# inhavl-shlee/AFI-GAN

Hardware: AMD Instinct MI355X
Metric: stage1_G+D_step_images_per_s (higher is better)
Workload: dtype f32 via f16x3: two scaled fp16 pieces per operand, three f16 MFMAs per product, fp32 accumulate (tensors fp32)

## Files before the change

afigan_amd/csrc/afi_launch.h:

```cpp
#pragma once
#include "afi_common.h"

int afi_launch_pix_gemm(const AfiPixGemm& p, int b_rc, hipStream_t st);
int afi_launch_gemm_tn(const float* Q, const float* V, float* dU, int planes, long long rows_per_plane, int M, int N, hipStream_t st, bool deterministic = false);
int afi_launch_gemm_nt(const float* A, const float* B, float* C, int planes, long long rows_per_plane, int N, int K, hipStream_t st);
int afi_launch_split_bf16_tiles(const float* B, void* out, int planes, int N, int K, int split, hipStream_t st);
int afi_launch_gemm_nt_bf16_dma(const float* A, const void* Bsplit, float* C, int planes, long long rows_per_plane, int N, int K, int split, hipStream_t st);
int afi_launch_gemm_tn_bf16(const float* Q, const float* V, float* dU, int planes, long long rows_per_plane, int M, int N, int split, hipStream_t st, bool deterministic = false);
int afi_launch_split_f16_tiles(const float* B, void* out, int planes, int N, int K, hipStream_t st, int wkind = 0);
int afi_f16_image_begin(void* out, hipStream_t st);
float* afi_f16_image_wmax(void* out);
long long afi_f16_image_bytes(int planes, int N, int K);
int afi_launch_absmax_planes(const float* X, long long per_plane, int planes, float* out, hipStream_t st);
AfiF16Bound afi_f16_bound(const float* amax, int kind);
int afi_launch_gemm_nt_f16x3(const float* A, const void* Bimg, float* C, int planes, long long rows_per_plane, int N, int K, const AfiF16Bound& ab, hipStream_t st,
                             bool a_pre = false, long long nt256_min_tiles = 512, bool local_sums = false);
int afi_launch_gemm_tn_f16x3(const float* Q, const float* V, float* dU, int planes, long long rows_per_plane, int M, int N, const AfiF16Bound& qb, const AfiF16Bound& vb,
                             hipStream_t st, bool pre = false, bool deterministic = false);
int afi_launch_wgrad_gemm(const AfiWgradGemm& p, hipStream_t st);
int afi_launch_wgrad_gemm_group(const AfiWgradGemm* probs, int n, int wide, hipStream_t st);
int afi_launch_wgrad_gemm_group6(const AfiWgradGemm* probs, int n, hipStream_t st);
int afi_launch_pix_gemm_group(const AfiPixGemm* probs, int n, int b_rc, hipStream_t st);

long long afi_wk6_image_bytes(int Ncols, int Ck, int ntaps, int nKphase);
int afi_launch_wk6_images(const AfiWk6ImgJob* jobs, int n, hipStream_t st, const AfiWk6Side* side = nullptr, const AfiWk6ConvT* ct = nullptr);
int afi_launch_rdb_chain6(const AfiChain6& c, hipStream_t st);
int afi_launch_pix_gemm_sk(const AfiPixGemm& p, int b_rc, hipStream_t st);
int afi_launch_pix_gemm_wk_group(const AfiPixGemm* probs, int n, int b_rc, hipStream_t st);
int afi_launch_wgrad_group(const AfiWgradGemm* probs, int n, int wide, hipStream_t st);
int afi_launch_wgrad6_group(const AfiWgradGemm* probs, int n, hipStream_t st);

int afi_launch_nchw_to_nhwc(const float* in, float* out, int N, int C, int P, hipStream_t st);
int afi_launch_cast_to_f32_nhwc(const void* in, int dt, int N, int C, int H, int W, long long sN, long long sC, long long sH, long long sW, float* out,
                                hipStream_t st);
int afi_launch_cast_from_f32_nhwc(const AfiView& in, int N, int H, int W, int C, void* out, int dt, hipStream_t st);

int afi_launch_colsum_group(const AfiColsumProb* probs, int n, hipStream_t st);
int afi_launch_nhwc_to_nchw(const float* in, float* out, int N, int C, int P, hipStream_t st);
int afi_launch_convT_pack(const float* W, float* Wp, int Cin, int Cout, hipStream_t st);
int afi_launch_convT_unpack_grad(const float* dWp, float* dW, int Cin, int Cout, hipStream_t st);
int afi_launch_rdb_wgrad_unpack(const float* dWp, float* const dw[4], int C, int G, float alpha, hipStream_t st);
int afi_launch_rdb_wgrad_unpack_multi(const float* dWp, long long stride, float* const (*dw)[4], int nblocks, int C, int G, float alpha, hipStream_t st);
int afi_launch_g_bwd_tail(const AfiColsumProb* cs, int n_cs, const float* dWpT, float* dWT, int Cin, int Cout,
                          const float* dWp, long long stride, float* const (*dw)[4], int nblocks, int C, int G, float alpha, hipStream_t st);
int afi_launch_rdb_xpart_pack(const float* const w[4], float* out, int C, int G, hipStream_t st);
int afi_launch_lrelu_slice(AfiView v, int N, int H, int W, int nch, hipStream_t st);
int afi_launch_bn_stats(const float* x, long long P, int C, float* mean, float* invstd, float* var_out, float* running_mean,
                        float* running_var, float* scratch, hipStream_t st, long long* num_batches_tracked = nullptr, float eps = -1.f,
                        float momentum = -1.f, bool fp64 = true);
int afi_launch_bn_stats_from_partials(const double* partial, int rows, long long P, int C, float* mean, float* invstd, float* var_out, float* running_mean,
                                      float* running_var, hipStream_t st, long long* num_batches_tracked = nullptr, float eps = -1.f, float momentum = -1.f);
int afi_launch_view_absmax(AfiView x, int N, int H, int W, int C, float* amax, hipStream_t st);
int afi_launch_bn_act_amax(const float* mm, int rows, int C, const float* mean, const float* invstd, const float* gamma, const float* beta, float slope,
                           float* amax, hipStream_t st);
int afi_launch_bn_apply_lrelu(const float* x, float* y, const float* mean, const float* invstd, const float* gamma, const float* beta,
                              long long P, int C, hipStream_t st, float slope = AFI_LRELU_SLOPE, float* amax = nullptr);
int afi_launch_bn_bwd(const float* g, const float* x, float* dx, const float* mean, const float* invstd, const float* gamma, float* dgamma,
                      float* dbeta, float gscale, long long P, int C, float* scratch, hipStream_t st, const float* mask_beta = nullptr,
                      float slope = AFI_LRELU_SLOPE, float* amax = nullptr);
int afi_launch_colsum_accum(const float* g, long long P, int C, long long ld, float alpha, float* db, float* scratch, hipStream_t st);
int afi_launch_bn_bwd_sums(const float* g, const float* x, const float* mean, const float* invstd, float* dgamma, float* dbeta, float* sums2C, long long P, int C,
                           float* scratch, hipStream_t st);
int afi_launch_bn_bwd_apply(const float* g, const float* x, float* dx, const float* mean, const float* invstd, const float* gamma, const float* sums2C, long long P,
                            long long P_total, int C, hipStream_t st);
int afi_launch_stencil9_sum(const float* d9, int ld, const float* bias, float* out, int N, int H, int W, hipStream_t st);
int afi_launch_stencil9_scatter(const float* dlogit, float* dd9, int ld, int N, int H, int W, hipStream_t st);
int afi_launch_bn_bwd_from_partials(const double* partial, int rows, const float* g, const float* x, float* dx, const float* mean, const float* invstd,
                                    const float* gamma, float* dgamma, float* dbeta, float gscale, long long P, int C, float* scratch, hipStream_t st,
                                    const float* mask_beta, float slope, float* amax);
extern "C" long long afi_disc_tail_scratch_floats(int C);
int afi_launch_disc_tail_fwd(const float* x, const AfiBnLoad* bn, float slope, const float* w3, float* d9, long long P, int C, hipStream_t st);
int afi_launch_disc_tail_bwd(const float* x, const float* dd9, const AfiBnLoad bn, float slope, const float* w3, float* dx, float* dgamma, float* dbeta, float* dw3,
                             long long P, int C, float* scratch, float* amax, hipStream_t st);
int afi_launch_bce_logits(const float* z, long long n, float target, float lscale, float* loss, float gscale, float* dz, hipStream_t st);
int afi_launch_l1(AfiView a, AfiView b, int N, int h, int w, int C, int Ha, int Wa, float lscale, float* loss, float gscale, float* da,
// ... 32 lines not shown
```

afigan_amd/csrc/igemm.hip:

```cpp
#include "afi_common.h"
#include "afi_launch.h"

#define AFI_BK 32
#define AFI_LDK (AFI_BK + 4)


__device__ __attribute__((aligned(16))) float afi_zeros[4] = {0.f, 0.f, 0.f, 0.f};

#include "afi_epilogue.h"

template <bool POST>
__global__ __launch_bounds__(256) void afi_pix_splitk_epilogue_kernel(const AfiPixGemm p) {
    const int HW = p.H * p.W;
    const long long M = (long long)p.N * HW;
    const int ldp = (p.Ncols + 3) & ~3;
    const int C_F4 = ldp >> 2;
    const long long total = M * C_F4;
    for (long long it = (long long)blockIdx.x * 256 + threadIdx.x; it < total; it += (long long)gridDim.x * 256) {
        const long long m = it / C_F4;
        const int col = (int)(it - m * C_F4) * 4;
        f32x4 v = {0.f, 0.f, 0.f, 0.f};
        const float* src = p.partial + m * ldp + col;
        const long long slab = M * ldp;
        int ks = 0;
// ... 479 lines not shown
    const long long ldn = p.N;
    if (use_atomic) {
#pragma unroll
        for (int mi = 0; mi < MI; ++mi)
#pragma unroll
            for (int r = 0; r < 16; ++r) {
                const int row = m0 + MI * ((r & 3) + 8 * (r >> 2) + 4 * lh) + mi;
                atomicAdd(out + (long long)row * ldn + n0 + wn * 32 + lr, acc[mi][r]);
            }
    } else {
        float old[MI][16];
#pragma unroll
        for (int mi = 0; mi < MI; ++mi)
#pragma unroll
            for (int r = 0; r < 16; ++r) {
                const int row = m0 + MI * ((r & 3) + 8 * (r >> 2) + 4 * lh) + mi;
                old[mi][r] = out[(long long)row * ldn + n0 + wn * 32 + lr];
            }
#pragma unroll
        for (int mi = 0; mi < MI; ++mi)
#pragma unroll
            for (int r = 0; r < 16; ++r) {
                const int row = m0 + MI * ((r & 3) + 8 * (r >> 2) + 4 * lh) + mi;
                out[(long long)row * ldn + n0 + wn * 32 + lr] = old[mi][r] + acc[mi][r];
            }
    }
}

#include <vector>
#include <atomic>
#include <mutex>
namespace {
struct ProfRec { hipEvent_t a, b; int kind; double flops; long long m; int n, k, split, planes; };
struct ProfState {
    std::atomic<bool> on{false};
    std::mutex mu;
    std::vector<ProfRec> recs;
    std::vector<hipEvent_t> pool;
    size_t used = 0;
} g_prof;
const char* kKindNames[] = {
    "pix_gemm<128x128,KC,linear> (1x1 / ragged-map / non-aligned Winograd GEMMs)", "pix_gemm<128x64,KC>", "pix_gemm<128x32,KC>", "pix_gemm<64x64,KC>",
    "pix_gemm<128x128,RC,linear> (conv dgrad, mid-size / ragged maps)", "pix_gemm<128x64,RC>", "pix_gemm<128x32,RC>", "pix_gemm<64x64,RC>",
    "wgrad_gemm<128x128>", "wgrad_gemm<64x128>", "wgrad_gemm<32x128>",
    "pix_gemm<128x128,KC,halo> (conv fwd)", "pix_gemm<128x128,RC,halo> (conv dgrad)",
    "gemm_nt<128x128> (batched Winograd GEMM)", "gemm_tn<128x128> (Winograd weight-gradient GEMM)",
    "pix_gemm_wk (small-map pixel GEMM, K split inside the block; grouped launches included)",
    "wgrad_group (grouped weight gradients of a small-map backward pass)",
    "gemm_nt_bf16<128x128> (batched Winograd GEMM on the bf16 MFMA: bf16x6 / bf16x3 / bf16 operands, fp32 accumulate)",
    "gemm_tn_bf16<128x128> (Winograd weight-gradient GEMM on the bf16 MFMA: bf16x6 / bf16x3 / bf16 operands, fp32 accumulate)",
    "wgrad_group6 (grouped weight gradients of a small-map backward pass on the bf16 MFMA, bf16x6 operands, fp32 accumulate)",
    "pix_gemm_wk6 (small-map pixel GEMM on the bf16 MFMA, bf16x6 operands on pre-split weight images, fp32 accumulate; grouped launches included)",
    "gemm_nt_f16x3 (batched Winograd GEMM on the f16 MFMA, 256x256 tiles where the grid fills the chip and 128x128 below: two scaled fp16 pieces per operand, three products, fp32 accumulate)",
    "gemm_tn_f16x3<128x128> (Winograd weight-gradient GEMM on the f16 MFMA: two scaled fp16 pieces per operand, three products, fp32 accumulate)"};
constexpr int kNumKinds = 23;
hipEvent_t prof_event() {
    if (g_prof.used == g_prof.pool.size()) {
        hipEvent_t e;
        (void)hipEventCreate(&e);
        g_prof.pool.push_back(e);
    }
    return g_prof.pool[g_prof.used++];
}
struct ProfScope {
    hipStream_t st; int kind; double flops; hipEvent_t a{};
    long long m = 0; int n = 0, k = 0, split = 1, planes = 1;
    ProfScope(hipStream_t s, int kd, double f) : st(s), kind(kd), flops(f) {
        if (g_prof.on) { std::lock_guard<std::mutex> lk(g_prof.mu); a = prof_event(); (void)hipEventRecord(a, st); started = true; }
    }
    bool live = true, started = false;
    void cancel() { live = false; }
    ~ProfScope() {
        if (started && live) { std::lock_guard<std::mutex> lk(g_prof.mu); hipEvent_t b = prof_event(); (void)hipEventRecord(b, st); g_prof.recs.push_back({a, b, kind, flops, m, n, k, split, planes}); }
    }
};
}

extern "C" int afi_profile_enable(int on) {
    std::lock_guard<std::mutex> lk(g_prof.mu);
    if (on) { g_prof.recs.clear(); g_prof.used = 0; }
    g_prof.on = on != 0;
    return AFI_OK;
}
extern "C" int afi_profile_num_kinds(void) { return kNumKinds; }
extern "C" const char* afi_profile_kind_name(int kind) { return (kind >= 0 && kind < kNumKinds) ? kKindNames[kind] : ""; }
extern "C" int afi_profile_get(int kind, double* out) {
    out[0] = out[1] = out[2] = 0.0;
    for (const ProfRec& r : g_prof.recs) {
        if (r.kind != kind) continue;
        if (hipEventSynchronize(r.b) != hipSuccess) return AFI_ERR_LAUNCH;
        float ms = 0.f;
        if (hipEventElapsedTime(&ms, r.a, r.b) != hipSuccess) return AFI_ERR_LAUNCH;
        out[0] += 1.0; out[1] += ms; out[2] += r.flops;
    }
    return AFI_OK;
}

#include <stdio.h>
extern "C" int afi_profile_dump(const char* path) {
    FILE* f = fopen(path, "w");
    if (!f) return AFI_ERR_BAD_ARG;
    fprintf(f, "kind,rows,cols,k,split,planes,ms,tflops\n");
    for (const ProfRec& r : g_prof.recs) {
        float ms = 0.f;
        if (hipEventSynchronize(r.b) != hipSuccess || hipEventElapsedTime(&ms, r.a, r.b) != hipSuccess) { fclose(f); return AFI_ERR_LAUNCH; }
        fprintf(f, "\"%s\",%lld,%d,%d,%d,%d,%.4f,%.2f\n", kKindNames[r.kind], r.m, r.n, r.k, r.split, r.planes, ms, ms > 0.f ? r.flops / (ms * 1e-3) / 1e12 : 0.0);
    }
    fclose(f);
// ... 224 lines not shown
            const long long blocks = tiles * s2;
            if (blocks < 2 * slots && s2 < maxsplit) continue;
            if (blocks > AFI_TN_MAX_ROUNDS * slots && best >= 0.0) break;
            const long long rounds = (blocks + slots - 1) / slots;
            const double fill = (double)blocks / (double)(rounds * slots);
            if (fill > best + 1e-3) { best = fill; splitK = s2; }
        }
    }
    if (deterministic) splitK = 1;
    int kper = (int)((rows_per_plane + splitK - 1) / splitK);
    kper = ((kper + 31) / 32) * 32;
    splitK = (int)((rows_per_plane + kper - 1) / kper);
    AfiGemmTN g{Q, V, dU, rows_per_plane, planes, M, N};
    ProfScope prof(st, 22, 2.0 * (double)rows_per_plane * planes * M * N);
    prof.m = (long long)M * planes; prof.n = N; prof.k = (int)rows_per_plane; prof.split = splitK; prof.planes = planes;
    if (pre) hipLaunchKernelGGL(afi_gemm_tn_f16x3_pre_kernel, dim3((unsigned)tiles, splitK), dim3(64 * AFI_TN_WAVES), (unsigned)AFI_TN_RING * 4u * 4096u, st, g, qb, vb, ntm, ntn, kper);
    else hipLaunchKernelGGL(afi_gemm_tn_f16x3_kernel, dim3((unsigned)tiles, splitK), dim3(256), 2u * 4u * 4096u, st, g, qb, vb, ntm, ntn, kper);
    return hipGetLastError() == hipSuccess ? AFI_OK : AFI_ERR_LAUNCH;
}
int afi_launch_pix_gemm_group(const AfiPixGemm* probs, int n, int b_rc, hipStream_t st) {
    double fl = 0.0; long long m = 0; int nn = 0;
    for (int i = 0; i < n; ++i) AFI_TRY(afi_o16_refused(probs[i]));
    for (int i = 0; i < n; ++i) {
        const long long M = (long long)probs[i].N * probs[i].H * probs[i].W;
        fl += 2.0 * (double)M * probs[i].Ncols * probs[i].ntaps * probs[i].nKphase * probs[i].Ck;
        m = M; nn += probs[i].Ncols;
    }
    bool all6 = n > 0;
    for (int i = 0; i < n; ++i) all6 = all6 && probs[i].Bimg != nullptr;
    ProfScope prof(st, all6 ? 20 : 15, fl);
    prof.m = m; prof.n = nn; prof.k = n > 0 ? probs[0].ntaps * probs[0].nKphase * probs[0].Ck : 0;
    const int rc = afi_launch_pix_gemm_wk_group(probs, n, b_rc, st);
    if (rc == AFI_ERR_UNSUPPORTED) prof.cancel();
    return rc;
}
int afi_launch_wgrad_gemm_group(const AfiWgradGemm* probs, int n, int wide, hipStream_t st) {
    if (n <= 0) return AFI_OK;
    double fl = 0.0;
    for (int i = 0; i < n; ++i) fl += 2.0 * (double)probs[i].N * probs[i].H * probs[i].W * probs[i].Mrows * probs[i].Ncols * probs[i].ntaps;
    ProfScope prof(st, 16, fl);
    prof.m = n;
    return afi_launch_wgrad_group(probs, n, wide, st);
}
int afi_launch_wgrad_gemm_group6(const AfiWgradGemm* probs, int n, hipStream_t st) {
    if (n <= 0) return AFI_OK;
    double fl = 0.0;
    for (int i = 0; i < n; ++i) fl += 2.0 * (double)probs[i].N * probs[i].H * probs[i].W * probs[i].Mrows * probs[i].Ncols * probs[i].ntaps;
    ProfScope prof(st, 19, fl);
    prof.m = n; prof.split = 6;
    const int rc = afi_launch_wgrad6_group(probs, n, st);
    if (rc == AFI_ERR_UNSUPPORTED) prof.cancel();
    return rc;
}
int afi_launch_pix_gemm(const AfiPixGemm& p_in, int b_rc, hipStream_t st) {
    AfiPixGemm p = p_in;
    const long long M = (long long)p.N * p.H * p.W;
    if (M <= 0 || p.Ncols <= 0 || p.Ck <= 0) return AFI_ERR_BAD_ARG;
    AFI_TRY(afi_o16_refused(p));
    if (p.a_bn.mean) return AFI_ERR_UNSUPPORTED;
    if (p.b_sImg != 0 && ((long long)p.H * p.W) % 128 != 0) return AFI_ERR_BAD_ARG;
    if (b_rc && (p.Ncols & 3)) return AFI_ERR_UNSUPPORTED;
    if (!b_rc && (p.Ck & 3)) return AFI_ERR_UNSUPPORTED;
    if (p.gtap) {
        if (p.ntaps < 1 || p.ntaps > 9 || p.a_sgn != 1 || p.nKphase != 1 || (p.a_stride != 1 && p.a_stride != 2)) return AFI_ERR_BAD_ARG;
        const bool small = M <= 64 * 256 || p.Ncols <= 64;
        if (!b_rc) return small ? launch_pix<64, 64, 2, 2, false, AFI_BK, false, true>(p, st) : launch_pix<128, 128, 2, 2, false, AFI_BK, false, true>(p, st);
        return small ? launch_pix<64, 64, 2, 2, true, AFI_BK, false, true>(p, st) : launch_pix<128, 128, 2, 2, true, AFI_BK, false, true>(p, st);
    }
    if (p.ntaps != 1 && p.ntaps != 9) return AFI_ERR_BAD_ARG;
    const bool smallM = (long long)afi_cdiv(M, 128) * afi_cdiv(p.Ncols, 128) < 128;
    if (smallM && p.b_sImg == 0) {
        ProfScope prof(st, p.Bimg ? 20 : 15, 2.0 * (double)M * p.Ncols * p.ntaps * p.nKphase * p.Ck);
        prof.m = M; prof.n = p.Ncols; prof.k = p.ntaps * p.nKphase * p.Ck;
        const int rc = afi_launch_pix_gemm_sk(p, b_rc, st);
        if (rc != AFI_ERR_UNSUPPORTED || p.Bimg) return rc;
        prof.cancel();
    }
    if (!p.B) return AFI_ERR_UNSUPPORTED;
    const long long padded = (long long)p.N * afi_cdiv(p.H, AFI_HALO_TY) * AFI_HALO_TY * afi_cdiv(p.W, AFI_HALO_TX) * AFI_HALO_TX;
    const bool halo = p.ntaps == 9 && p.nKphase == 1 && p.a_up == 1 && !smallM && p.Ncols > 64 && padded * 100 <= M * 112;
    if (!b_rc) {
        if (p.Ncols <= 32) return launch_pix<128, 32, 4, 1, false>(p, st);
        if (p.Ncols <= 64) return smallM ? launch_pix<64, 64, 2, 2, false>(p, st) : launch_pix<128, 64, 2, 2, false>(p, st);
        if (smallM) return launch_pix<64, 64, 2, 2, false>(p, st);
        if (halo) return launch_pix<128, 128, 2, 2, false, 32, true>(p, st);
        return launch_pix<128, 128, 2, 2, false>(p, st);
    } else {
        if (p.Ncols <= 32) return launch_pix<128, 32, 4, 1, true>(p, st);
        if (p.Ncols <= 64) return smallM ? launch_pix<64, 64, 2, 2, true>(p, st) : launch_pix<128, 64, 2, 2, true>(p, st);
        if (smallM) return launch_pix<64, 64, 2, 2, true>(p, st);
        if (halo) return launch_pix<128, 128, 2, 2, true, 32, true>(p, st);
        return launch_pix<128, 128, 2, 2, true>(p, st);
    }
}

template <int BM, int BN, int WM, int WN>
static int launch_wgrad(const AfiWgradGemm& p, hipStream_t st) {
    const long long P = (long long)p.N * p.H * p.W;
    const int ntm = afi_cdiv(p.Mrows, BM), ntn = afi_cdiv(p.Ncols, BN);
    const long long tiles = (long long)ntm * ntn * p.ntaps;
    int splitK = p.splitK;
    if (splitK <= 0) {
        splitK = 1;
        const long long want = 1024;
        if (tiles < want) splitK = (int)((want + tiles - 1) / tiles);
        const int maxsplit = (int)((P + 8 * AFI_BK - 1) / (8 * AFI_BK));
// ... 103 lines not shown
```

afigan_amd/csrc/nets.hip:

```cpp
#include <string.h>
#include <stdlib.h>

#include "../../include/afigan_hip.h"
#include "afi_common.h"
#include "afi_launch.h"
#include <initializer_list>
#include <new>


#include <vector>
namespace {
struct SideStream {
    hipStream_t side = nullptr;
    std::vector<hipEvent_t> ring;
    size_t next = 0;
    bool init() {
        if (side) return true;
        if (hipStreamCreateWithFlags(&side, hipStreamNonBlocking) != hipSuccess) { side = nullptr; return false; }
        ring.resize(128);
        for (auto& e : ring)
            if (hipEventCreateWithFlags(&e, hipEventDisableTiming) != hipSuccess) return false;
        return true;
    }
    void destroy() {
        for (auto& e : ring) if (e) (void)hipEventDestroy(e);
        ring.clear();
        if (side) (void)hipStreamDestroy(side);
        side = nullptr;
    }
    hipEvent_t ev() { hipEvent_t e = ring[next]; next = (next + 1) % ring.size(); return e; }
};
struct WinoWeightCache {
    float* buf = nullptr;
    long long floats = 0, used = 0;
    struct Entry { const float* w; int f4, mode, O, I; long long off; } e[128];
    int n = 0;
};
struct WinoWgradAccum {
    float* buf = nullptr;
    long long floats = 0, used = 0;
    struct Entry { float* dw; int f4, O, I; float alpha; long long off; } e[64];
    int n = 0;
};
}
struct AfiOptions { long long v[AFI_OPT_COUNT]; };
#ifndef AFI_DEFAULT_LOCAL_SUMS
#define AFI_DEFAULT_LOCAL_SUMS 12
#endif
#ifndef AFI_DEFAULT_F4_FORWARD
#define AFI_DEFAULT_F4_FORWARD 12
#endif
static const AfiOptions kDefaultOptions = {{ 1,  1,  AFI_DEFAULT_F4_FORWARD,  1,  1024,
                                             2048,  2048,  3000,
                                             1,  4096,  0,  0,  0,  1,  512,
                                             AFI_DEFAULT_LOCAL_SUMS,  1,  0}};
struct afi_ctx {
    int device = -1;
    float* op_scratch = nullptr; long long op_scratch_floats = 0;
    int dtype = AFI_DTYPE_DEFAULT;
    AfiOptions opt = kDefaultOptions;
    WinoWeightCache wcache;
    WinoWgradAccum wgacc;
    SideStream side;
    struct AmaxPool { float* p = nullptr; int next = 0; } amax[2];
};
static inline long long afi_opt(const afi_ctx* cx, int o) { return cx ? cx->opt.v[o] : kDefaultOptions.v[o]; }
static inline int afi_default_dtype() { return AFI_DTYPE_DEFAULT; }

static inline bool afi_dtype_ok(int d) { return d == AFI_DTYPE_F32 || d == AFI_DTYPE_BF16 || d == AFI_DTYPE_F16X3 || d == AFI_DTYPE_BF16X3 || d == AFI_DTYPE_BF16X6; }
static inline bool afi_dtype_smallmap6(int d) { return d == AFI_DTYPE_BF16X6 || d == AFI_DTYPE_F16X3; }
namespace {
struct Fork {
    afi_ctx* cx; hipStream_t main, side;
    bool on;
    Fork(afi_ctx* c, hipStream_t m, bool enable) : cx(c), main(m), side(m), on(false) {
        if (enable && cx && cx->side.init()) { side = cx->side.side; on = true; after_main(); }
    }
    ~Fork() { join(); }
    void after_main() {
        if (!on) return;
        hipEvent_t e = cx->side.ev();
        if (hipEventRecord(e, main) != hipSuccess || hipStreamWaitEvent(side, e, 0) != hipSuccess) { on = false; side = main; }
    }
    void join() {
        if (!on) return;
        hipEvent_t e = cx->side.ev();
        (void)hipEventRecord(e, side);
        (void)hipStreamWaitEvent(main, e, 0);
        on = false;
    }
};
constexpr long long kSideStreamMaxPixels = 12000;
}
#define AFI_CTX_CHECK(ctx) do { if (ctx) { int d_ = -1; if (hipGetDevice(&d_) != hipSuccess || d_ != ((afi_ctx*)(ctx))->device) return AFI_ERR_BAD_ARG; \
                                           ((afi_ctx*)(ctx))->amax[0].p = ((afi_ctx*)(ctx))->amax[1].p = nullptr; } } while (0)

static inline bool afi_det(const afi_ctx* cx) { return afi_opt(cx, AFI_OPT_DETERMINISTIC) != 0; }
static inline int wgrad_launch(const afi_ctx* cx, AfiWgradGemm g, hipStream_t st) {
    if (afi_det(cx)) g.splitK = 1;
    return afi_launch_wgrad_gemm(g, st);
}
static inline int launch_pix_op(afi_ctx* cx, AfiPixGemm g, int b_rc, hipStream_t st) {
    if (cx && cx->op_scratch && !g.partial) { g.partial = cx->op_scratch; g.partial_floats = cx->op_scratch_floats; }
    return afi_launch_pix_gemm(g, b_rc, st);
}
static inline AfiView V(afi_view_t v) { return AfiView{v.p, v.sN, v.sH, v.sW}; }
static inline AfiView dense_view(const float* p, int H, int W, long long ld) {
    return AfiView{const_cast<float*>(p), (long long)H * W * ld, (long long)W * ld, ld};
}
static inline AfiView ch_off(AfiView v, long long c) { v.p += c; return v; }
static inline AfiView null_view() { return AfiView{nullptr, 0, 0, 0}; }
static inline long long align4(long long n) { return (n + 3) & ~3LL; }

static AfiPixGemm pix_default(int N, int H, int W) {
    AfiPixGemm g;
    memset(&g, 0, sizeof(g));
    g.N = N; g.H = H; g.W = W;
    g.ntaps = 9; g.nKphase = 1; g.a_sgn = 1; g.a_up = 1; g.o_up = 1;
    g.alpha = 1.f; g.beta = 0.f; g.r1s = 1.f; g.r2s = 1.f;
    g.a_stride = 1; g.aH = H; g.aW = W; g.oH = g.oW = 1 << 30; g.post_scale = 1.f;
    return g;
}

static AfiPixGemm conv_fwd_desc(AfiView x, int N, int H, int W, int Cin, const float* w, const float* bias, int Cout, AfiView out) {
    AfiPixGemm g = pix_default(N, H, W);
    g.Ck = Cin; g.Ncols = Cout; g.CoutPhase = Cout;
    g.A = x; g.B = w; g.b_sRow = 9LL * Cin; g.b_sTap = Cin;
    g.O = out; g.bias = bias;
    return g;
}
static AfiPixGemm conv_dgrad_desc(AfiView dy, int N, int H, int W, int Cout, const float* w, int Cin, AfiView dx) {
    AfiPixGemm g = pix_default(N, H, W);
    g.a_sgn = -1;
    g.Ck = Cout; g.Ncols = Cin; g.CoutPhase = Cin;
    g.A = dy; g.B = w; g.b_sRow = 9LL * Cin; g.b_sTap = Cin;
    g.O = dx;
    return g;
}
static AfiWgradGemm conv_wgrad_desc(AfiView dy, AfiView x, int N, int H, int W, int Cout, int Cin, float* dw, float alpha) {
    AfiWgradGemm g;
    memset(&g, 0, sizeof(g));
    g.N = N; g.H = H; g.W = W; g.ntaps = 9;
    g.Mrows = Cout; g.Ncols = Cin;
    g.DY = dy; g.dy_up = 1; g.CoutPhase = Cout;
// ... 545 lines not shown
}
int afi_conv3x3_wgrad(afi_ctx_t* ctx, afi_view_t dy, afi_view_t x, int N, int H, int W, int Cout, int Cin, float* dw, float alpha, void* stream) {
    afi_ctx* cx = ctx; (void)cx;
    AFI_CTX_CHECK(ctx);
    if ((Cin & 3) || (Cout & 3)) return AFI_ERR_UNSUPPORTED;
    return wgrad_launch(cx, conv_wgrad_desc(V(dy), V(x), N, H, W, Cout, Cin, dw, alpha), (hipStream_t)stream);
}

long long afi_conv3x3_wino_ws_floats(int N, int H, int W, int Cin, int Cout) { return wino_ws_floats(N, H, W, Cin, Cout); }
int afi_conv3x3_wino_fwd(afi_ctx_t* ctx, afi_view_t x, int N, int H, int W, int Cin, const float* w, const float* bias, int Cout, afi_view_t out, float* ws,
                         long long ws_floats, void* stream) {
    afi_ctx* cx = ctx; (void)cx;
    AFI_CTX_CHECK(ctx);
    if (N <= 0 || H <= 0 || W <= 0 || !ws) return AFI_ERR_BAD_ARG;
    return wino_conv(cx, kWinoFwd, V(x), N, H, W, Cin, w, Cout, bias, V(out), null_view(), ws, ws_floats, nullptr, 0, (hipStream_t)stream);
}
int afi_conv3x3_wino_fwd_out16(afi_ctx_t* ctx, afi_view_t x, int N, int H, int W, int Cin, const float* w, const float* bias, int Cout, afi_view_t out,
                               int out_dtype, float* ws, long long ws_floats, void* stream) {
    afi_ctx* cx = ctx; (void)cx;
    AFI_CTX_CHECK(ctx);
    if (out_dtype != AFI_STORE_BF16 && out_dtype != AFI_STORE_F16) return AFI_ERR_BAD_ARG;
    if (N <= 0 || H <= 0 || W <= 0 || !ws) return AFI_ERR_BAD_ARG;
    if ((Cin & 3) || (Cout & 3)) return AFI_ERR_UNSUPPORTED;
    AfiPixGemm g = conv_fwd_desc(V(x), N, H, W, Cin, w, bias, Cout, V(out));
    g.o_dtype = out_dtype;
    return wino_run(cx, g, wino_form(cx, g, 0), ws, ws_floats, nullptr, 0, (hipStream_t)stream);
}
int afi_conv3x3_wino_infer(afi_ctx_t* ctx, afi_view_t x, int N, int H, int W, int Cin, const float* w, const float* bias, int Cout, afi_view_t out, int act,
                           float* ws, long long ws_floats, void* stream) {
    afi_ctx* cx = ctx; (void)cx;
    AFI_CTX_CHECK(ctx);
    if (N <= 0 || H <= 0 || W <= 0 || !ws || act < 0 || act > 2) return AFI_ERR_BAD_ARG;
    if ((Cin & 3) || (Cout & 3)) return AFI_ERR_UNSUPPORTED;
    AfiPixGemm g = conv_fwd_desc(V(x), N, H, W, Cin, w, bias, Cout, V(out));
    g.lrelu = act;
    return wino_run(cx, g, wino_form(cx, g, 0, true), ws, ws_floats, nullptr, 0, (hipStream_t)stream);
}
int afi_conv3x3_wino_dgrad(afi_ctx_t* ctx, afi_view_t dy, int N, int H, int W, int Cout, const float* w, int Cin, afi_view_t dx, afi_view_t z, float* ws,
                           long long ws_floats, void* stream) {
    afi_ctx* cx = ctx; (void)cx;
    AFI_CTX_CHECK(ctx);
    if (N <= 0 || H <= 0 || W <= 0 || !ws) return AFI_ERR_BAD_ARG;
    return wino_conv(cx, kWinoDgrad, V(dy), N, H, W, Cout, w, Cin, nullptr, V(dx), z.p ? V(z) : null_view(), ws, ws_floats, nullptr, 0, (hipStream_t)stream);
}

int afi_conv3x3_wino_wgrad(afi_ctx_t* ctx, afi_view_t dy, afi_view_t x, int N, int H, int W, int Cout, int Cin, float* dw, float alpha, float* ws,
                           long long ws_floats, void* stream) {
    afi_ctx* cx = ctx; (void)cx;
    AFI_CTX_CHECK(ctx);
    if (N <= 0 || H <= 0 || W <= 0 || !ws || !dw) return AFI_ERR_BAD_ARG;
    return wino_wgrad(cx, V(dy), V(x), N, H, W, Cout, Cin, dw, alpha, ws, ws_floats, (hipStream_t)stream);
}

int afi_conv1x1_fwd(afi_ctx_t* ctx, afi_view_t x, int N, int H, int W, int Cin, const float* w, const float* bias, int Cout, afi_view_t out, float alpha,
                    float beta, afi_view_t r1, float r1_scale, int lrelu, void* stream) {
    afi_ctx* cx = ctx; (void)cx;
    AFI_CTX_CHECK(ctx);
    if ((Cin & 3) || (Cout & 3)) return AFI_ERR_UNSUPPORTED;
    AfiPixGemm g = pix_default(N, H, W);
    g.ntaps = 1; g.Ck = Cin; g.Ncols = Cout; g.CoutPhase = Cout;
    g.A = V(x); g.B = w; g.b_sRow = Cin; g.b_sTap = 0;
    g.O = V(out); g.bias = bias; g.alpha = alpha; g.beta = beta; g.lrelu = lrelu;
    if (r1.p) { g.R1 = V(r1); g.r1s = r1_scale; g.r1_lo = 0; g.r1_hi = Cout; }
    return launch_pix_op(cx, g, 0, (hipStream_t)stream);
}
int afi_conv1x1_dgrad(afi_ctx_t* ctx, afi_view_t dy, int N, int H, int W, int Cout, const float* w, int Cin, afi_view_t dx, float alpha, float beta,
                      void* stream) {
    afi_ctx* cx = ctx; (void)cx;
    AFI_CTX_CHECK(ctx);
    if ((Cin & 3) || (Cout & 3)) return AFI_ERR_UNSUPPORTED;
    AfiPixGemm g = pix_default(N, H, W);
    g.ntaps = 1; g.a_sgn = -1; g.Ck = Cout; g.Ncols = Cin; g.CoutPhase = Cin;
    g.A = V(dy); g.B = w; g.b_sRow = Cin; g.b_sTap = 0;
    g.O = V(dx); g.alpha = alpha; g.beta = beta;
    return launch_pix_op(cx, g, 1, (hipStream_t)stream);
}
int afi_conv1x1_dgrad_out16(afi_ctx_t* ctx, afi_view_t dy, int N, int H, int W, int Cout, const float* w, int Cin, afi_view_t dx, int dx_dtype, float alpha,
                            float beta, void* stream) {
    afi_ctx* cx = ctx; (void)cx;
    AFI_CTX_CHECK(ctx);
    if (dx_dtype != AFI_STORE_BF16 && dx_dtype != AFI_STORE_F16) return AFI_ERR_BAD_ARG;
    if ((Cin & 3) || (Cout & 3)) return AFI_ERR_UNSUPPORTED;
    AfiPixGemm g = pix_default(N, H, W);
    g.ntaps = 1; g.a_sgn = -1; g.Ck = Cout; g.Ncols = Cin; g.CoutPhase = Cin;
    g.A = V(dy); g.B = w; g.b_sRow = Cin; g.b_sTap = 0;
    g.O = V(dx); g.alpha = alpha; g.beta = beta; g.o_dtype = dx_dtype;
    return launch_pix_op(cx, g, 1, (hipStream_t)stream);
}
int afi_conv1x1_wgrad(afi_ctx_t* ctx, afi_view_t dy, afi_view_t x, int N, int H, int W, int Cout, int Cin, float* dw, float alpha, void* stream) {
    afi_ctx* cx = ctx; (void)cx;
    AFI_CTX_CHECK(ctx);
    if ((Cin & 3) || (Cout & 3)) return AFI_ERR_UNSUPPORTED;
    AfiWgradGemm g = conv_wgrad_desc(V(dy), V(x), N, H, W, Cout, Cin, dw, alpha);
    g.ntaps = 1; g.dw_sRow = Cin; g.dw_sTap = 0;
    return wgrad_launch(cx, g, (hipStream_t)stream);
}

int afi_conv3x3s2_fwd(afi_ctx_t* ctx, afi_view_t x, int N, int Hi, int Wi, int Cin, const float* w, const float* bias, int Cout, afi_view_t out, int act,
                      afi_view_t act_out, float post_scale, afi_view_t r, float r_scale, void* stream) {
    afi_ctx* cx = ctx; (void)cx;
    AFI_CTX_CHECK(ctx);
    if ((Cin & 3) || (Cout & 3)) return AFI_ERR_UNSUPPORTED;
    if (Hi < 1 || Wi < 1) return AFI_ERR_BAD_ARG;
    const int Ho = (Hi + 1) / 2, Wo = (Wi + 1) / 2;
    AfiPixGemm g = conv_fwd_desc(V(x), N, Ho, Wo, Cin, w, bias, Cout, V(out));
    g.gtap = 1; g.a_stride = 2; g.aH = Hi; g.aW = Wi;
    for (int t = 0; t < 9; ++t) { g.tap_dy[t] = (signed char)(t / 3 - 1); g.tap_dx[t] = (signed char)(t % 3 - 1); g.tap_w[t] = (signed char)t; }
    g.lrelu = act; g.r2_post = 1; g.post_scale = post_scale;
    if (act_out.p) g.O2 = V(act_out);
    if (r.p) { g.R2 = V(r); g.r2s = r_scale; g.r2_lo = 0; g.r2_hi = Cout; }
    return launch_pix_op(cx, g, 0, (hipStream_t)stream);
}
int afi_conv3x3s2_dgrad(afi_ctx_t* ctx, afi_view_t dy, int N, int Hi, int Wi, int Cout, const float* w, int Cin, afi_view_t dx, float alpha, float beta,
                        void* stream) {
    afi_ctx* cx = ctx; (void)cx;
    AFI_CTX_CHECK(ctx);
// ... 1107 lines not shown
```

include/afigan_hip.h:

```cpp
#ifndef AFIGAN_HIP_H
#define AFIGAN_HIP_H

#include <stddef.h>
#include <stdint.h>

#ifdef __cplusplus
extern "C" {
#endif

#define AFI_OK 0
#define AFI_ERR_BAD_ARG 1
#define AFI_ERR_UNSUPPORTED 2
#define AFI_ERR_LAUNCH 3
#define AFI_ERR_WORKSPACE 4

#define AFI_MAX_RDB 8

typedef struct afi_view {
    float* p;
    long long sN, sH, sW;
} afi_view_t;

int afi_abi_version(void);
const char* afi_status_string(int status);

typedef struct afi_ctx afi_ctx_t;
const char* afi_build_id(void);
int afi_ctx_create(afi_ctx_t** out);
int afi_ctx_destroy(afi_ctx_t* ctx);
int afi_ctx_set_op_scratch(afi_ctx_t* ctx, float* scratch, long long floats);
#define AFI_DTYPE_F32 0
#define AFI_DTYPE_BF16 1
#define AFI_DTYPE_F16X3 2
#define AFI_DTYPE_BF16X3 3
#define AFI_DTYPE_BF16X6 6
#define AFI_DTYPE_DEFAULT AFI_DTYPE_F16X3
int afi_ctx_set_compute_dtype(afi_ctx_t* ctx, int dtype);
int afi_ctx_get_compute_dtype(const afi_ctx_t* ctx);
#define AFI_OPT_WINOGRAD 0
#define AFI_OPT_WINOGRAD_F4_BACKWARD 1
#define AFI_OPT_WINOGRAD_F4_FORWARD 2
#define AFI_OPT_BN_STATS_FP64 3
#define AFI_OPT_D_WINOGRAD_MIN_PIXELS 4
#define AFI_OPT_G_WINOGRAD_MIN_PIXELS 5
#define AFI_OPT_G_SMALLMAP_MAX_PIXELS 6
#define AFI_OPT_G_GROUPED_WGRAD_MAX_PIXELS 7
#define AFI_OPT_G_BATCH_GROWTH_GRADS 8
#define AFI_OPT_G_SMALLMAP6_MAX_PIXELS 9
#define AFI_OPT_G_RDB_CHAIN 10
#define AFI_OPT_D_FOLD_BN_APPLY 11
#define AFI_OPT_DETERMINISTIC 12
#define AFI_OPT_F16_PRESPLIT 13
#define AFI_OPT_F16_NT256_MIN_TILES 14
#define AFI_OPT_F16_LOCAL_SUMS 15
#define AFI_OPT_D_FUSE_TAIL 16
#define AFI_OPT_D_FUSE_BWD_SUMS 17
#define AFI_OPT_COUNT 18
int afi_ctx_set_option(afi_ctx_t* ctx, int option, long long value);
long long afi_ctx_get_option(const afi_ctx_t* ctx, int option);
long long afi_gemm_nt_scratch_bytes(int planes, int N, int K, int dtype);
int afi_gemm_nt(const float* A, const float* B, float* C, int planes, long long rows_per_plane, int N, int K, int dtype, void* scratch,
                long long scratch_bytes, void* stream);
long long afi_gemm_tn_scratch_bytes(int planes, int dtype);
int afi_gemm_tn(const float* Q, const float* V, float* dU, int planes, long long rows_per_plane, int M, int N, int dtype, void* scratch,
                long long scratch_bytes, void* stream);
int afi_ctx_set_wino_weight_cache(afi_ctx_t* ctx, float* buf, long long floats);
int afi_ctx_wino_weight_cache_invalidate(afi_ctx_t* ctx);
int afi_ctx_set_wino_wgrad_accum(afi_ctx_t* ctx, float* buf, long long floats);
int afi_ctx_wino_wgrad_flush(afi_ctx_t* ctx, void* stream);
int afi_ctx_wino_wgrad_discard(afi_ctx_t* ctx);


typedef struct afi_gen_params {
    int C;
    int G;
    int n_rdb;
    float residual_scale;
    float* w0; float* b0;
    float* rdb_w[AFI_MAX_RDB][5];
    float* w7; float* b7;
    float* wT; float* bT;
    float* w9; float* b9;
} afi_gen_params_t;

long long afi_generator_fwd_ws_floats(int C, int G, int n_rdb, int N, int H, int W);
long long afi_generator_bwd_ws_floats(int C, int G, int n_rdb, int N, int H, int W);

int afi_generator_fwd(afi_ctx_t* ctx, const afi_gen_params_t* prm, afi_view_t x, int N, int H, int W, afi_view_t out,
                      float* ws, long long ws_floats, void* stream);
int afi_generator_bwd(afi_ctx_t* ctx, const afi_gen_params_t* prm, const afi_gen_params_t* grads, afi_view_t x, int N, int H, int W,
                      const float* ws, const float* dout, float* dx, float* scratch, long long scratch_floats, void* stream);

#define AFI_STORE_F32 0
#define AFI_STORE_BF16 1
#define AFI_STORE_F16 2
int afi_generator_fwd_out16(afi_ctx_t* ctx, const afi_gen_params_t* prm, afi_view_t x, int N, int H, int W, afi_view_t out, int out_dtype,
                            float* ws, long long ws_floats, void* stream);

typedef struct afi_disc_params {
    int F[4];
    float* w[3]; float* b[3];
    float* gamma[3]; float* beta[3];
    float* running_mean[3]; float* running_var[3];
    long long* num_batches_tracked[3];
    float* w3; float* b3;
} afi_disc_params_t;

long long afi_discriminator_fwd_ws_floats(const int F[4], int N, int H, int W);
long long afi_discriminator_fwd_ws_floats_ex(const afi_ctx_t* ctx, const int F[4], int N, int H, int W, int training);
long long afi_discriminator_bwd_ws_floats(const int F[4], int N, int H, int W);
int afi_discriminator_ws_layout(const int F[4], int N, int H, int W, long long* off12);
int afi_discriminator_saved_activations(const afi_ctx_t* ctx, const int F[4], int N, int H, int W);
// ... 176 lines not shown
```

Measured before the change: 28.66.

## Add persistent fp32-MFMA streaming kernel for large-map forward 1x1 convs

New measurement: 28.59. About the same (-0.3%).

```diff
diff --git a/afigan_amd/csrc/afi_launch.h b/afigan_amd/csrc/afi_launch.h
--- a/afigan_amd/csrc/afi_launch.h
+++ b/afigan_amd/csrc/afi_launch.h
@@ -21,6 +21,11 @@
 int afi_launch_wgrad_gemm_group(const AfiWgradGemm* probs, int n, int wide, hipStream_t st);
 int afi_launch_wgrad_gemm_group6(const AfiWgradGemm* probs, int n, hipStream_t st);
 int afi_launch_pix_gemm_group(const AfiPixGemm* probs, int n, int b_rc, hipStream_t st);
+
+int afi_launch_conv1x1_stream(const AfiPixGemm& p, hipStream_t st);
+
+bool afi_conv1x1_stream_takes(const AfiPixGemm& p);
+int afi_launch_conv1x1_stream_kernels(const AfiPixGemm& p, hipStream_t st);
 
 long long afi_wk6_image_bytes(int Ncols, int Ck, int ntaps, int nKphase);
 int afi_launch_wk6_images(const AfiWk6ImgJob* jobs, int n, hipStream_t st, const AfiWk6Side* side = nullptr, const AfiWk6ConvT* ct = nullptr);
diff --git a/afigan_amd/csrc/conv1x1_stream.hip b/afigan_amd/csrc/conv1x1_stream.hip
--- /dev/null
+++ b/afigan_amd/csrc/conv1x1_stream.hip
@@ -0,0 +1,230 @@
+#include "afi_common.h"
+#include "afi_launch.h"
+#include "afi_epilogue.h"
+
+#define AFI_S_BM 128
+#define AFI_S_BK 32
+#define AFI_S_LDK (AFI_S_BK + 4)
+#define AFI_S_CPATCH (8 * AFI_S_LDK)
+
+static inline size_t afi_s_lds_bytes(int BN, int Cin, bool resident) {
+    const size_t w = resident ? (size_t)BN * (Cin + 4) : (size_t)2 * BN * AFI_S_LDK;
+    return sizeof(float) * (w + 2 * AFI_S_BM * AFI_S_LDK + 4 * AFI_S_CPATCH);
+}
+
+template <int BN>
+__global__ __launch_bounds__(256, 2) void afi_conv1x1_stream_kernel(const AfiPixGemm p, int n_base, int ntn, int ntm, int resident) {
+    constexpr int NI = BN / 64;
+    constexpr int B_LOADS = BN / 32;
+    extern __shared__ __attribute__((aligned(16))) float smem[];
+    const int tid = threadIdx.x, lane = tid & 63, wave = tid >> 6;
+    const int wm = wave >> 1, wn = wave & 1, lr = lane & 31, lh = lane >> 5;
+    const int aq = tid & 7, ar = tid >> 3;
+    const int K = p.Ck, nK = K / AFI_S_BK;
+    const int wpitch = resident ? K + 4 : AFI_S_LDK;
+    float* Wl = smem;
+    float* Al = smem + (resident ? BN * (K + 4) : 2 * BN * AFI_S_LDK);
+    float* Cl = Al + 2 * AFI_S_BM * AFI_S_LDK + wave * AFI_S_CPATCH;
+    const unsigned HW = (unsigned)(p.H * p.W), Wd = (unsigned)p.W;
+    const unsigned M = (unsigned)p.N * HW;
+
+    int u0, u1;
+    {
+        const int nwg = gridDim.x, q = nwg >> 3, r = nwg & 7, xcd = blockIdx.x & 7;
+        const long long L = (xcd < r ? xcd * (q + 1) : r * (q + 1) + (xcd - r) * q) + (int)(blockIdx.x >> 3);
+        const long long U = (long long)ntm * ntn;
+        u0 = (int)(L * U / nwg); u1 = (int)((L + 1) * U / nwg);
+    }
+    if (u0 >= u1) return;
+    auto unit_tm = [&](int u) { return resident ? u % ntm : u / ntn; };
+    auto unit_tn = [&](int u) { return resident ? u / ntm : u % ntn; };
+
+    int ld_u = u0, ld_k = 0;
+    long long a_off[4]; bool a_ok[4];
+    const float* b_row = p.B;
+    auto setup_loader = [&](int u) {
+        const unsigned m0 = (unsigned)unit_tm(u) * AFI_S_BM;
+#pragma unroll
+        for (int i = 0; i < 4; ++i) {
+            const unsigned m = m0 + ar + 32 * i;
+            a_ok[i] = m < M;
+            const unsigned mm = a_ok[i] ? m : 0u;
+            const unsigned img = mm / HW, rem = mm - img * HW, y = rem / Wd, x = rem - y * Wd;
+            a_off[i] = (long long)img * p.A.sN + (long long)y * p.A.sH + (long long)x * p.A.sW + 4 * aq;
+        }
+        b_row = p.B + (long long)(n_base + unit_tn(u) * BN + ar) * p.b_sRow + 4 * aq;
+    };
+    f32x4 a_reg[4], b_reg[B_LOADS];
+    auto load_stage = [&]() {
+        const int c0 = ld_k * AFI_S_BK;
+#pragma unroll
+        for (int i = 0; i < 4; ++i) {
+            f32x4 v = {0.f, 0.f, 0.f, 0.f};
+            if (a_ok[i]) v = *(const f32x4*)(p.A.p + (a_off[i] + c0));
+            a_reg[i] = v;
+        }
+        if (!resident) {
+#pragma unroll
+            for (int i = 0; i < B_LOADS; ++i) b_reg[i] = *(const f32x4*)(b_row + (long long)(32 * i) * p.b_sRow + c0);
+        }
+        if (++ld_k == nK) {
+            ld_k = 0;
+            if (++ld_u < u1) setup_loader(ld_u);
+        }
+    };
+    auto store_stage = [&](int buf) {
+        float* As = Al + buf * (AFI_S_BM * AFI_S_LDK);
+#pragma unroll
+        for (int i = 0; i < 4; ++i) *(f32x4*)(As + (ar + 32 * i) * AFI_S_LDK + 4 * aq) = a_reg[i];
+        if (!resident) {
+            float* Ws = Wl + buf * (BN * AFI_S_LDK);
+#pragma unroll
+            for (int i = 0; i < B_LOADS; ++i) *(f32x4*)(Ws + (ar + 32 * i) * AFI_S_LDK + 4 * aq) = b_reg[i];
+        }
+    };
+    auto load_panel = [&](int tn) {
+        const int k4 = K >> 2;
+        const float* src = p.B + (long long)(n_base + tn * BN) * p.b_sRow;
+        for (int it = tid; it < BN * k4; it += 256) {
+            const int n = it / k4, c4 = it - n * k4;
+            *(f32x4*)(Wl + n * wpitch + 4 * c4) = *(const f32x4*)(src + (long long)n * p.b_sRow + 4 * c4);
+        }
+    };
+
+    f32x16 acc[2][NI];
+    auto zero_acc = [&]() {
+#pragma unroll
+        for (int mi = 0; mi < 2; ++mi)
+#pragma unroll
+            for (int ni = 0; ni < NI; ++ni)
+#pragma unroll
+                for (int r = 0; r < 16; ++r) acc[mi][ni][r] = 0.f;
+    };
+    auto compute_stage = [&](int buf, int ck) {
+        const float* As = Al + buf * (AFI_S_BM * AFI_S_LDK) + ((wm * 2) * 32 + lr) * AFI_S_LDK + lh * 4;
+        const float* Bs = (resident ? Wl + ck * AFI_S_BK : Wl + buf * (BN * AFI_S_LDK)) + ((wn * NI) * 32 + lr) * wpitch + lh * 4;
+#pragma unroll
+        for (int s = 0; s < AFI_S_BK / 8; ++s) {
+            f32x4 fa[2], fb[NI];
+#pragma unroll
+            for (int mi = 0; mi < 2; ++mi) fa[mi] = *(const f32x4*)(As + mi * 32 * AFI_S_LDK + s * 8);
+#pragma unroll
+            for (int ni = 0; ni < NI; ++ni) fb[ni] = *(const f32x4*)(Bs + ni * 32 * wpitch + s * 8);
+            __builtin_amdgcn_s_setprio(1);
+#pragma unroll
+            for (int j = 0; j < 4; ++j)
+#pragma unroll
+                for (int mi = 0; mi < 2; ++mi)
+#pragma unroll
+                    for (int ni = 0; ni < NI; ++ni)
+                        acc[mi][ni] = __builtin_amdgcn_mfma_f32_32x32x2f32(fa[mi][j], fb[ni][j], acc[mi][ni], 0, 0, 0);
+            __builtin_amdgcn_s_setprio(0);
+        }
+    };
+    auto epilogue = [&](int u) {
+        const unsigned m0 = (unsigned)unit_tm(u) * AFI_S_BM + wm * 64 + (lane >> 3);
+        const int col0 = n_base + unit_tn(u) * BN + wn * (BN / 2) + 4 * (lane & 7);
+#pragma unroll
+        for (int mi = 0; mi < 2; ++mi)
+#pragma unroll
+            for (int q = 0; q < 4; ++q) {
+                const unsigned m = m0 + mi * 32 + 8 * q;
+                const bool ok = m < M;
+                const unsigned mm = ok ? m : 0u;
+                const unsigned img = mm / HW, rem = mm - img * HW, y = rem / Wd, x = rem - y * Wd;
+#pragma unroll
+                for (int ni = 0; ni < NI; ++ni) {
+#pragma unroll
+                    for (int r = 0; r < 4; ++r) Cl[(r + 4 * lh) * AFI_S_LDK + lr] = acc[mi][ni][4 * q + r];
+                    __builtin_amdgcn_fence(__ATOMIC_RELEASE, "wavefront");
+                    __builtin_amdgcn_wave_barrier();
+                    const f32x4 v = *(const f32x4*)(Cl + (lane >> 3) * AFI_S_LDK + 4 * (lane & 7));
+                    __builtin_amdgcn_fence(__ATOMIC_ACQUIRE, "wavefront");
+                    __builtin_amdgcn_wave_barrier();
+                    if (ok) afi_epilogue_store<false>(p, (int)img, (int)y, (int)x, col0 + ni * 32, v);
+                }
+            }
+    };
+
+    int cu = u0, ck = 0, panel_tn = -1;
+    setup_loader(u0);
+    load_stage();
+    zero_acc();
+    for (int g = 0;; ++g) {
+        const int buf = g & 1;
+        if (resident && ck == 0 && unit_tn(cu) != panel_tn) {
+            __syncthreads();
+            panel_tn = unit_tn(cu);
+            load_panel(panel_tn);
+        }
+        store_stage(buf);
+        __syncthreads();
+        if (ld_u < u1) load_stage();
+        compute_stage(buf, ck);
+        if (++ck == nK) {
+            epilogue(cu);
+            ck = 0;
+            if (++cu == u1) break;
+            zero_acc();
+        }
+    }
+}
+
+#include <mutex>
+#include <set>
+#include <utility>
+static bool afi_s_opt_in_lds(const void* fn) {
+    static std::mutex mu;
+    static std::set<std::pair<int, const void*>> done;
+    int dev = -1;
+    if (hipGetDevice(&dev) != hipSuccess) return false;
+    std::lock_guard<std::mutex> lk(mu);
+    if (done.count({dev, fn})) return true;
+    if (hipFuncSetAttribute(fn, hipFuncAttributeMaxDynamicSharedMemorySize, 160 * 1024) != hipSuccess) return false;
+    done.insert({dev, fn});
+    return true;
+}
+
+static int afi_s_cu_count() {
+    static std::mutex mu;
+    static int cached[64] = {0};
+    int dev = -1;
+    if (hipGetDevice(&dev) != hipSuccess || dev < 0) return 0;
+    std::lock_guard<std::mutex> lk(mu);
+    if (dev < 64 && cached[dev] > 0) return cached[dev];
+    int cus = 0;
+    if (hipDeviceGetAttribute(&cus, hipDeviceAttributeMultiprocessorCount, dev) != hipSuccess) return 0;
+    if (dev < 64) cached[dev] = cus;
+    return cus;
+}
+
+template <int BN>
+static int launch_stream(const AfiPixGemm& p, int n_base, int ntn, hipStream_t st) {
+    const long long M = (long long)p.N * p.H * p.W;
+    const int ntm = afi_cdiv(M, AFI_S_BM);
+    const bool resident = afi_s_lds_bytes(BN, p.Ck, true) <= 80 * 1024;
+    const size_t lds = afi_s_lds_bytes(BN, p.Ck, resident);
+    if (lds > 160 * 1024) return AFI_ERR_UNSUPPORTED;
+    if (lds > 64 * 1024 && !afi_s_opt_in_lds((const void*)afi_conv1x1_stream_kernel<BN>)) return AFI_ERR_LAUNCH;
+    const int cus = afi_s_cu_count();
+    if (cus <= 0) return AFI_ERR_LAUNCH;
+    long long grid = (long long)cus * (lds <= 80 * 1024 ? 2 : 1);
+    const long long units = (long long)ntm * ntn;
+    if (grid > units) grid = units;
+    hipLaunchKernelGGL((afi_conv1x1_stream_kernel<BN>), dim3((unsigned)grid), dim3(256), lds, st, p, n_base, ntn, ntm, resident ? 1 : 0);
+    return hipGetLastError() == hipSuccess ? AFI_OK : AFI_ERR_LAUNCH;
+}
+
+bool afi_conv1x1_stream_takes(const AfiPixGemm& p) {
+    const long long M = (long long)p.N * p.H * p.W;
+    return p.ntaps == 1 && p.nKphase == 1 && !p.gtap && p.a_sgn == 1 && p.a_up == 1 && p.o_up == 1 && p.b_sImg == 0 && p.B && !p.a_bn.mean &&
+           p.o_dtype == AFI_STORE_F32 && !p.r2_post && !p.stats && !p.stats_mm && !p.bstats && p.Ck > 0 && p.Ck % AFI_S_BK == 0 &&
+           p.Ncols > 0 && p.Ncols % 64 == 0 && p.CoutPhase == p.Ncols && M > 0 && M < (1LL << 31) - AFI_S_BM;
+}
+int afi_launch_conv1x1_stream_kernels(const AfiPixGemm& p, hipStream_t st) {
+    if (!afi_conv1x1_stream_takes(p)) return AFI_ERR_UNSUPPORTED;
+    const int n128 = p.Ncols / 128, rem64 = (p.Ncols % 128) / 64;
+    if (n128) AFI_TRY(launch_stream<128>(p, 0, n128, st));
+    if (rem64) AFI_TRY(launch_stream<64>(p, n128 * 128, 1, st));
+    return AFI_OK;
+}
diff --git a/afigan_amd/csrc/igemm.hip b/afigan_amd/csrc/igemm.hip
--- a/afigan_amd/csrc/igemm.hip
+++ b/afigan_amd/csrc/igemm.hip
@@ -555,8 +555,9 @@
     "wgrad_group6 (grouped weight gradients of a small-map backward pass on the bf16 MFMA, bf16x6 operands, fp32 accumulate)",
     "pix_gemm_wk6 (small-map pixel GEMM on the bf16 MFMA, bf16x6 operands on pre-split weight images, fp32 accumulate; grouped launches included)",
     "gemm_nt_f16x3 (batched Winograd GEMM on the f16 MFMA, 256x256 tiles where the grid fills the chip and 128x128 below: two scaled fp16 pieces per operand, three products, fp32 accumulate)",
-    "gemm_tn_f16x3<128x128> (Winograd weight-gradient GEMM on the f16 MFMA: two scaled fp16 pieces per operand, three products, fp32 accumulate)"};
-constexpr int kNumKinds = 23;
+    "gemm_tn_f16x3<128x128> (Winograd weight-gradient GEMM on the f16 MFMA: two scaled fp16 pieces per operand, three products, fp32 accumulate)",
+    "conv1x1_stream (persistent fp32-MFMA GEMM of the forward 1x1 conv on maps of >= 32768 pixels; a 64-column remainder launch included)"};
+constexpr int kNumKinds = 24;
 hipEvent_t prof_event() {
     if (g_prof.used == g_prof.pool.size()) {
         hipEvent_t e;
@@ -887,6 +888,14 @@
     if (rc == AFI_ERR_UNSUPPORTED) prof.cancel();
     return rc;
 }
+int afi_launch_conv1x1_stream(const AfiPixGemm& p, hipStream_t st) {
+    const long long M = (long long)p.N * p.H * p.W;
+    ProfScope prof(st, 23, 2.0 * (double)M * p.Ncols * p.Ck);
+    prof.m = M; prof.n = p.Ncols; prof.k = p.Ck;
+    const int rc = afi_launch_conv1x1_stream_kernels(p, st);
+    if (rc == AFI_ERR_UNSUPPORTED) prof.cancel();
+    return rc;
+}
 int afi_launch_pix_gemm(const AfiPixGemm& p_in, int b_rc, hipStream_t st) {
     AfiPixGemm p = p_in;
     const long long M = (long long)p.N * p.H * p.W;
diff --git a/afigan_amd/csrc/nets.hip b/afigan_amd/csrc/nets.hip
--- a/afigan_amd/csrc/nets.hip
+++ b/afigan_amd/csrc/nets.hip
@@ -59,6 +59,7 @@
     float* op_scratch = nullptr; long long op_scratch_floats = 0;
     int dtype = AFI_DTYPE_DEFAULT;
     AfiOptions opt = kDefaultOptions;
+    bool conv1x1_stream = true;
     WinoWeightCache wcache;
     WinoWgradAccum wgacc;
     SideStream side;
@@ -90,6 +91,7 @@
         on = false;
     }
 };
+constexpr long long kConv1x1StreamMinPixels = 32768;
 constexpr long long kSideStreamMaxPixels = 12000;
 }
 #define AFI_CTX_CHECK(ctx) do { if (ctx) { int d_ = -1; if (hipGetDevice(&d_) != hipSuccess || d_ != ((afi_ctx*)(ctx))->device) return AFI_ERR_BAD_ARG; \
@@ -741,6 +743,13 @@
     return wino_wgrad(cx, V(dy), V(x), N, H, W, Cout, Cin, dw, alpha, ws, ws_floats, (hipStream_t)stream);
 }
 
+int afi_ctx_set_conv1x1_stream(afi_ctx_t* ctx, int on) {
+    if (!ctx || (on != 0 && on != 1)) return AFI_ERR_BAD_ARG;
+    ctx->conv1x1_stream = on != 0;
+    return AFI_OK;
+}
+int afi_ctx_get_conv1x1_stream(const afi_ctx_t* ctx) { return ctx ? (ctx->conv1x1_stream ? 1 : 0) : 1; }
+
 int afi_conv1x1_fwd(afi_ctx_t* ctx, afi_view_t x, int N, int H, int W, int Cin, const float* w, const float* bias, int Cout, afi_view_t out, float alpha,
                     float beta, afi_view_t r1, float r1_scale, int lrelu, void* stream) {
     afi_ctx* cx = ctx; (void)cx;
@@ -751,6 +760,9 @@
     g.A = V(x); g.B = w; g.b_sRow = Cin; g.b_sTap = 0;
     g.O = V(out); g.bias = bias; g.alpha = alpha; g.beta = beta; g.lrelu = lrelu;
     if (r1.p) { g.R1 = V(r1); g.r1s = r1_scale; g.r1_lo = 0; g.r1_hi = Cout; }
+    if ((!cx || cx->conv1x1_stream) && (long long)N * H * W >= kConv1x1StreamMinPixels && Cin % 32 == 0 && Cout % 64 == 0 &&
+        afi_conv1x1_stream_takes(g))
+        return afi_launch_conv1x1_stream(g, (hipStream_t)stream);
     return launch_pix_op(cx, g, 0, (hipStream_t)stream);
 }
 int afi_conv1x1_dgrad(afi_ctx_t* ctx, afi_view_t dy, int N, int H, int W, int Cout, const float* w, int Cin, afi_view_t dx, float alpha, float beta,
diff --git a/include/afigan_hip.h b/include/afigan_hip.h
--- a/include/afigan_hip.h
+++ b/include/afigan_hip.h
@@ -58,6 +58,8 @@
 #define AFI_OPT_COUNT 18
 int afi_ctx_set_option(afi_ctx_t* ctx, int option, long long value);
 long long afi_ctx_get_option(const afi_ctx_t* ctx, int option);
+int afi_ctx_set_conv1x1_stream(afi_ctx_t* ctx, int on);
+int afi_ctx_get_conv1x1_stream(const afi_ctx_t* ctx);
 long long afi_gemm_nt_scratch_bytes(int planes, int N, int K, int dtype);
 int afi_gemm_nt(const float* A, const float* B, float* C, int planes, long long rows_per_plane, int N, int K, int dtype, void* scratch,
                 long long scratch_bytes, void* stream);
```
